# ChampiB/CBO_with_OOP

Measured on AMD Instinct MI355X. Metric: candidate-intervention acquisitions/sec (16k grid, d=3), higher is better.
Workload: dtype f64

## Files before the change

cbo_with_oop_amd/_lib.py:

```python
from __future__ import annotations

import atexit
import ctypes
import os
import threading
import weakref

import numpy as np

_HERE = os.path.dirname(os.path.abspath(__file__))
LIB_PATH = os.environ.get("CBO_HIP_LIB", os.path.join(_HERE, "libcbo_hip.so"))

c_double_p = ctypes.POINTER(ctypes.c_double)
c_int64_p = ctypes.POINTER(ctypes.c_int64)
c_int_p = ctypes.POINTER(ctypes.c_int)
c_void_pp = ctypes.POINTER(ctypes.c_void_p)

ABI_VERSION = 5
ABI_DIAG_BASE = 1000
MAX_DIM = 8
CBO_OK = 0
CBO_ERR_INVALID = -1
CBO_ERR_HIP = -2
CBO_ERR_NOT_PD = -3
# ... 79 lines not shown
                                        c_double_p, ctypes.c_int64, c_void_pp]),
    "cbo_cands_destroy": (None, [ctypes.c_void_p]),
    "cbo_cands_keep_solution": (ctypes.c_int, [ctypes.c_void_p, ctypes.c_int]),
    "cbo_gp_append": (ctypes.c_int, [ctypes.c_void_p, c_double_p, ctypes.c_double, ctypes.c_double, ctypes.c_double,
                                     c_int_p]),
    "cbo_acq_sweep": (ctypes.c_int, [ctypes.c_void_p, ctypes.c_void_p, ctypes.c_double, ctypes.c_int,
                                     ctypes.c_double, ctypes.c_double, c_double_p, c_double_p, c_double_p,
                                     c_double_p, c_int64_p]),
    "cbo_gp_fit_sweep": (ctypes.c_int, [ctypes.c_void_p, ctypes.c_void_p, ctypes.c_double, ctypes.c_int,
                                        ctypes.c_double, ctypes.c_double, c_double_p, c_double_p, c_double_p,
                                        c_double_p, c_int64_p, c_int_p, c_double_p]),
    "cbo_acq_sweep_sets": (ctypes.c_int, [ctypes.c_int, c_void_pp, c_void_pp, c_double_p, ctypes.c_int, ctypes.c_double,
                                          c_double_p, c_double_p, c_int64_p]),
    "cbo_gp_fit_level": (ctypes.c_int, [ctypes.c_void_p, ctypes.c_int, c_int_p, c_double_p]),
    "cbo_comm_gather_i64": (ctypes.c_int, [ctypes.c_void_p, ctypes.c_int64, c_int64_p]),
    "cbo_comm_share_factor": (ctypes.c_int, [ctypes.c_void_p, ctypes.c_void_p, ctypes.c_int, c_int_p, ctypes.c_int,
                                              c_int_p, ctypes.c_int]),
    "cbo_gp_take_factor_slices": (ctypes.c_int, [ctypes.c_void_p, ctypes.c_void_p, ctypes.c_int, ctypes.c_int]),
    "cbo_schedule_report": (ctypes.c_int, [ctypes.c_void_p, ctypes.c_char_p, ctypes.c_int64]),
    "cbo_trial_step": (ctypes.c_int, [ctypes.c_int, c_void_pp, c_void_pp, ctypes.c_int, ctypes.c_int64, c_double_p, c_double_p,
                                      c_double_p, c_double_p, c_double_p, ctypes.c_int, ctypes.c_double, c_double_p, c_double_p,
                                      c_int64_p, c_int_p]),
    "cbo_acq_sweep_host": (ctypes.c_int, [ctypes.c_void_p, ctypes.c_int64, c_double_p, c_double_p, c_double_p,
                                          ctypes.c_double, ctypes.c_int, ctypes.c_double, ctypes.c_double,
                                          c_double_p, c_double_p, c_int64_p]),
    "cbo_argmax_sets": (ctypes.c_int, [c_double_p, ctypes.c_int, c_int_p]),
    "cbo_argmax_pairs": (ctypes.c_int, [c_double_p, c_int64_p, ctypes.c_int, c_double_p, c_int64_p]),
    "cbo_sem_create": (ctypes.c_int, [ctypes.c_void_p, ctypes.POINTER(CboSemSpec), ctypes.c_int64, ctypes.c_int,
                                      c_double_p, c_void_pp]),
    "cbo_sem_destroy": (None, [ctypes.c_void_p]),
    "cbo_sem_target": (ctypes.c_int, [ctypes.c_void_p, ctypes.c_int, ctypes.c_int64, ctypes.c_int, c_int_p,
                                      c_double_p, c_double_p]),
    "cbo_selftest_mfma": (ctypes.c_int, [ctypes.c_void_p, c_double_p]),
    "cbo_comm_unique_id": (ctypes.c_int, [ctypes.c_void_p]),
    "cbo_comm_init_rank": (ctypes.c_int, [ctypes.c_void_p, ctypes.c_int, ctypes.c_int, ctypes.c_void_p, c_void_pp]),
    "cbo_comm_init_all": (ctypes.c_int, [ctypes.c_int, c_void_pp, c_void_pp]),
    "cbo_comm_destroy": (None, [ctypes.c_void_p]),
    "cbo_comm_size": (ctypes.c_int, [ctypes.c_void_p, c_int_p, c_int_p]),
    "cbo_comm_argmax": (ctypes.c_int, [ctypes.c_void_p, ctypes.c_double, ctypes.c_int64, c_double_p, c_int64_p]),
    "cbo_comm_argmax_all": (ctypes.c_int, [ctypes.c_int, c_void_pp, c_double_p, c_int64_p, c_double_p, c_int64_p]),
    "cbo_comm_max_f64": (ctypes.c_int, [ctypes.c_void_p, ctypes.c_double, c_double_p]),
    "cbo_comm_barrier": (ctypes.c_int, [ctypes.c_void_p]),
}

_lib = None
_lock = threading.Lock()


def load():
    global _lib
    with _lock:
        if _lib is None:
            if not os.path.exists(LIB_PATH):
                raise ImportError(
                    f"{LIB_PATH} not found: build it with `make -C cbo_with_oop_amd/csrc` (or "
                    f"`python -c 'import __graft_entry__ as g; g.build()'`).  There is no CPU fallback.")
            lib = ctypes.CDLL(LIB_PATH)
            for name, (restype, argtypes) in SIGNATURES.items():
                fn = getattr(lib, name)
                fn.restype = restype
                fn.argtypes = argtypes
            version = lib.cbo_abi_version()
            if version >= ABI_DIAG_BASE and os.environ.get("CBO_HIP_ALLOW_DIAG") != "1":
                raise ImportError(
                    f"{LIB_PATH} is a timing-only diagnostic build (cbo_abi_version() = {version}): its results may be "
                    f"wrong by construction.  Measurement scripts opt in with CBO_HIP_ALLOW_DIAG=1.")
# ... 131 lines not shown
```

cbo_with_oop_amd/csrc/cbo_api.hip:

```cpp
#include <algorithm>
#include <atomic>
#include <cmath>
#include <cstdio>
#include <cstdlib>
#include <chrono>
#include <cstring>
#include <mutex>
#include <string>
#include <map>
#include <utility>
#include <vector>

#include "cbo_internal.h"
#include "schedule_tuner.h"

using namespace cbo;

static thread_local std::string g_err;
static std::atomic<uint64_t> g_fit_stamp{0};

static int fail(int code, const std::string &msg)
{
    g_err = msg;
    return code;
// ... 350 lines not shown
    if (c->sweep_stream) hipStreamDestroy(c->sweep_stream);
    if (c->bulk_stream) hipStreamDestroy(c->bulk_stream);
    if (c->side_stream) hipStreamDestroy(c->side_stream);
    if (c->stream) hipStreamDestroy(c->stream);
    delete c;
}

extern "C" int cbo_synchronize(cbo_ctx *c)
{
    if (!c) return fail(CBO_ERR_INVALID, "ctx is NULL");
    HIP_TRY(hipSetDevice(c->device));
    HIP_TRY(hipDeviceSynchronize());
    return CBO_OK;
}

#ifdef CBO_DIAG_KNOBS
__global__ void diag_fill_kernel(double *p, int64_t n)
{
    for (int64_t i = blockIdx.x * (int64_t)blockDim.x + threadIdx.x; i < n; i += (int64_t)gridDim.x * blockDim.x)
        p[i] = 1e-3 * (double)((i * 2654435761u) & 1023u) - 0.5;
}
extern "C" int cbo_diag_update_kernel_time(cbo_ctx *c, int n, int klen, int chunk_blocks, int half_lds, int upper, int reps,
                                           double *ms_out)
{
    if (!c || !ms_out) return fail(CBO_ERR_INVALID, "NULL argument");
    HIP_TRY(hipSetDevice(c->device));
    const int64_t lda = (int64_t)n + 80;
    double *A = nullptr;
    HIP_TRY(hipMalloc(&A, sizeof(double) * (size_t)n * (size_t)lda));
    hipLaunchKernelGGL(diag_fill_kernel, dim3(4096), dim3(256), 0, c->stream, A, (int64_t)n * lda);
    hipEvent_t a, b;
    HIP_TRY(hipEventCreate(&a));
    HIP_TRY(hipEventCreate(&b));
    launch_gemm_update(c->stream, A, lda, A, lda, A, lda, 0, klen, klen, n, n, chunk_blocks, half_lds != 0, upper != 0, nullptr);
    HIP_TRY(hipEventRecord(a, c->stream));
    for (int r = 0; r < reps; ++r)
        launch_gemm_update(c->stream, A, lda, A, lda, A, lda, 0, klen, klen, n, n, chunk_blocks, half_lds != 0, upper != 0, nullptr);
    HIP_TRY(hipEventRecord(b, c->stream));
    HIP_TRY(hipStreamSynchronize(c->stream));
    float ms = 0.f;
    HIP_TRY(hipEventElapsedTime(&ms, a, b));
    *ms_out = (double)ms / reps;
    hipEventDestroy(a);
    hipEventDestroy(b);
    hipFree(A);
    return CBO_OK;
}
#endif

extern "C" int cbo_set_profiling(cbo_ctx *c, int enabled)
{
    if (!c) return fail(CBO_ERR_INVALID, "ctx is NULL");
    c->profiling = enabled != 0;
    return CBO_OK;
}

extern "C" int cbo_reset_timers(cbo_ctx *c)
{
    if (!c) return fail(CBO_ERR_INVALID, "ctx is NULL");
    resolve_events(c);
    c->timers = cbo_timers{};
    return CBO_OK;
}

extern "C" int cbo_get_timers(cbo_ctx *c, cbo_timers *out)
{
    if (!c || !out) return fail(CBO_ERR_INVALID, "NULL argument");
    resolve_events(c);
    *out = c->timers;
    return CBO_OK;
// ... 1622 lines not shown
        const int frc = cbo_gp_fit(g, nullptr, nullptr);
        if (frc != CBO_OK) return frc;
    }
    int rc = ensure_alpha(g);
    if (rc != CBO_OK) return rc;
    const int64_t n_pad = g->n_pad;
    int64_t chunk = 0, ldv = 0;
    rc = ensure_workspaces(c, n_pad, n_pad, &chunk, &ldv);
    if (rc != CBO_OK) return rc;
    if (chunk < n_pad) return fail(CBO_ERR_UNSUPPORTED, "likelihood gradients need an n_pad x n_pad workspace (raise CBO_HIP_WORKSPACE_MB)");
    const int64_t ldw = n_pad + kLdExtra;
    const size_t w_bytes = sizeof(double) * (size_t)n_pad * (size_t)ldw;
    const size_t part_elems = (size_t)lml_grad_tiles(n_pad) * (size_t)(1 + g->d);
    if (w_bytes > c->W_bytes || part_elems > c->gpart_elems) {
        HIP_TRY(hipStreamSynchronize(c->stream));
        hipFree(c->W); hipFree(c->gpart);
        c->W = nullptr; c->gpart = nullptr; c->W_bytes = 0; c->gpart_elems = 0;
        HIP_TRY(hipMalloc(&c->W, w_bytes));
        c->W_bytes = w_bytes;
        HIP_TRY(hipMalloc(&c->gpart, sizeof(double) * part_elems));
        c->gpart_elems = part_elems;
    }
    launch_set_identity(c->stream, c->V, ldv, n_pad);
    if (prefer_right_looking(c, n_pad, n_pad)) {
        rc = enqueue_right_looking(g, c->V, ldv, n_pad, c->q, c->mu, true);
        if (rc != CBO_OK) return rc;
    } else {
        launch_trsm_strips(c->stream, g->A, g->lda, g->invDt, c->V, ldv, n_pad, n_pad, g->z, c->q, c->mu);
    }
    HIP_TRY(hipMemsetAsync(c->W, 0, w_bytes, c->stream));
    for (int k0 = 0; k0 < (int)n_pad; k0 += 256) {
        const int klen = (k0 + 256 <= (int)n_pad) ? 256 : 128;
        launch_gemm_update(c->stream, c->V, ldv, c->V, ldv, c->W, ldw, k0, klen, 0, k0 + klen, k0 + klen,
                           c->pipe_chunk_blocks, true, true);
    }
    launch_lml_grad(c->stream, g->X, g->h, g->alpha, c->W, ldw, n_pad, c->gpart, c->part_val);
    launch_lml_terms(c->stream, g->A, g->lda, n_pad, g->z, c->part_val + 16);
    HIP_TRY(hipGetLastError());
    launch_dot2(c->stream, g->alpha, g->alpha, g->n, c->part_val + 20);
    launch_sum(c->stream, c->q, g->n, c->part_val + 22);
    HIP_TRY(hipGetLastError());
    double hs[24];
    HIP_TRY(hipMemcpyAsync(hs, c->part_val, sizeof(hs), hipMemcpyDeviceToHost, c->stream));
    HIP_TRY(hipStreamSynchronize(c->stream));
    lml_outputs(g, hs, hs[16], hs[17], hs[20], hs[22], lml_out, dvariance_out, dlengthscale_out, dnoise_out);
    return CBO_OK;
}

static int ensure_reversed_factor(cbo_gp *g)
{
    cbo_ctx *c = g->ctx;
    if (!g->T) {
        HIP_TRY(hipMalloc(&g->T, sizeof(double) * (size_t)g->n_pad * (size_t)g->lda));
        HIP_TRY(hipMalloc(&g->invT, sizeof(double) * (size_t)(g->n_pad / 16) * 256));
        g->t_stamp = 0;
    }
    if (g->t_stamp != g->fit_stamp) {
        launch_reversed_factor(c->stream, g->A, g->lda, g->n_pad, g->invDt, g->T, g->lda, g->invT);
        HIP_TRY(hipGetLastError());
        g->t_stamp = g->fit_stamp;
    }
    return CBO_OK;
}

extern "C" int cbo_gp_predict_gradients(cbo_gp *g, int64_t m, const double *Xs, const double *pv_s, double *dmean_out,
                                        double *dvar_out)
{
// ... 229 lines not shown
    if (target < 0 || target >= m->spec.n_nodes) return fail(CBO_ERR_INVALID, "sem: target node out of range");
    if (n_iv < 0 || n_iv > CBO_SEM_MAX_NODES) return fail(CBO_ERR_INVALID, "sem: n_iv out of range");
    if (n_iv > 0 && (!iv_nodes || !values)) return fail(CBO_ERR_INVALID, "sem: intervention nodes/values missing");
    for (int j = 0; j < n_iv; ++j)
        if (iv_nodes[j] < 0 || iv_nodes[j] >= m->spec.n_nodes)
            return fail(CBO_ERR_INVALID, "sem: intervened node out of range");
    cbo_ctx *c = m->ctx;
    HIP_TRY(hipSetDevice(c->device));
    const int nb = sem_partial_blocks(m->n_draws);
    const int iv_cols = n_iv > 0 ? n_iv : 1;
    if (n_iv_sets > m->cap_m || iv_cols > m->cap_iv) {
        HIP_TRY(hipStreamSynchronize(c->stream));
        hipFree(m->values); hipFree(m->partial); hipFree(m->mean); hipFree(m->iv_nodes);
        m->values = m->partial = m->mean = nullptr; m->iv_nodes = nullptr; m->cap_m = 0; m->cap_iv = 0;
        const int64_t cap = n_iv_sets > m->cap_m ? n_iv_sets : m->cap_m;
        HIP_TRY(hipMalloc(&m->values, sizeof(double) * cap * CBO_SEM_MAX_NODES));
        HIP_TRY(hipMalloc(&m->partial, sizeof(double) * cap * nb));
        HIP_TRY(hipMalloc(&m->mean, sizeof(double) * cap));
        HIP_TRY(hipMalloc(&m->iv_nodes, sizeof(int) * CBO_SEM_MAX_NODES));
        m->cap_m = cap; m->cap_iv = CBO_SEM_MAX_NODES;
    }
    if (n_iv > 0) {
        HIP_TRY(hipMemcpyAsync(m->values, values, sizeof(double) * n_iv_sets * n_iv, hipMemcpyHostToDevice, c->stream));
        HIP_TRY(hipMemcpyAsync(m->iv_nodes, iv_nodes, sizeof(int) * n_iv, hipMemcpyHostToDevice, c->stream));
    }
    launch_sem_target(c->stream, m->spec, m->eps_cm, m->n_draws, target, n_iv_sets, n_iv, iv_nodes, m->iv_nodes, m->values,
                      m->partial, m->mean);
    HIP_TRY(hipGetLastError());
    HIP_TRY(hipMemcpyAsync(mean_out, m->mean, sizeof(double) * n_iv_sets, hipMemcpyDeviceToHost, c->stream));
    HIP_TRY(hipStreamSynchronize(c->stream));
    return CBO_OK;
}

extern "C" int cbo_selftest_mfma(cbo_ctx *c, double *max_abs_err_out)
{
    if (!c) return fail(CBO_ERR_INVALID, "ctx is NULL");
    HIP_TRY(hipSetDevice(c->device));
    double err = -1.0;
    if (run_mfma_selftest(c->stream, &err) != 0) return fail(CBO_ERR_HIP, "mfma selftest launch failed");
    if (max_abs_err_out) *max_abs_err_out = err;
    if (err != 0.0) return fail(CBO_ERR_HIP, "fp64 MFMA lane map differs from what the kernels assume");
    double err32 = -1.0;
    if (run_mfma_f32_selftest(c->stream, &err32) != 0) return fail(CBO_ERR_HIP, "f32 mfma selftest launch failed");
    if (max_abs_err_out) *max_abs_err_out = err32 > err ? err32 : err;
    if (err32 != 0.0) return fail(CBO_ERR_HIP, "fp32 MFMA lane map differs from what the kernels assume");
    return CBO_OK;
}
```

cbo_with_oop_amd/csrc/cbo_internal.h:

```cpp
#pragma once

#include <hip/hip_runtime.h>
#include <cstddef>
#include <cstdint>
#include <string>
#include <vector>

#include "cbo_hip.h"

namespace cbo {

typedef double d4 __attribute__((ext_vector_type(4)));
typedef double d2 __attribute__((ext_vector_type(2)));

#if defined(__HIP_DEVICE_COMPILE__) || defined(__HIPCC__)
typedef __attribute__((address_space(3))) void *lds_ptr_t;
__device__ __forceinline__ void glds16(const double *gsrc, unsigned lds_dst)
{
    unsigned keep;
    asm volatile("s_mov_b32 %0, m0\n\ts_mov_b32 m0, %2\n\ts_nop 0\n\tglobal_load_lds_dwordx4 %1, off\n\ts_mov_b32 m0, %0"
                 : "=&s"(keep)
                 : "v"(gsrc), "s"(lds_dst)
                 : "memory");
}
// ... 92 lines not shown
void set_panel_form_override(int form);
void sweep_pipe_pair(const SweepPipe &pipe, hipStream_t chain, const double *A, int64_t lda, const double *invDt,
                     int64_t n_pad, int p, int r0, int klen);
void sweep_pipe_tail(const SweepPipe &pipe, hipStream_t chain, const double *A, int64_t lda, const double *invDt,
                     int64_t n_pad, int pairs_done);
void launch_backsolve(hipStream_t s, const double *A, int64_t lda, int64_t n_pad, const double *invDt, double *alpha);
void launch_forward_vec(hipStream_t s, const double *A, int64_t lda, int64_t n_pad, const double *invDt, double *w,
                        double *out);
void launch_gather_column(hipStream_t s, const double *V, int64_t ldv, int64_t n_pad, double *dst);
bool launch_backsolve_chain(hipStream_t s, const double *A, int64_t lda, int64_t n_pad, const double *invDt,
                            const double *src, int64_t src_stride, double *work, double *out, int *info);
bool launch_forward_chain(hipStream_t s, const double *A, int64_t lda, int64_t n_pad, const double *invDt, const double *w,
                          double *out, int *info);
void launch_backsolve_vec(hipStream_t s, const double *A, int64_t lda, int64_t n_pad, const double *invDt,
                          const double *src, int64_t src_stride, double *work, double *out);
void launch_pred_gradients(hipStream_t s, const PointSet &X, int64_t n_pad, const PointSet &C, int64_t c_begin,
                           int64_t cols, int64_t m, const KernelHyper &h, const double *inv_ls_dev, const double *alpha,
                           const double *W, int64_t ldw, double *dmean, double *dvar);
void launch_reversed_factor(hipStream_t s, const double *A, int64_t lda, int64_t n_pad, const double *invDt, double *T,
                            int64_t ldt, double *invT);
void launch_reverse_rows(hipStream_t s, const double *V, int64_t ldv, int64_t n_pad, int64_t cols, double *W, int64_t ldw);
void launch_dot2(hipStream_t s, const double *a, const double *b, int64_t n, double *out2);
void launch_sum(hipStream_t s, const double *a, int64_t n, double *out);
void launch_expand_interventions(hipStream_t s, const double *observed, int64_t n_obs, int d, const double *values, int n_iv,
                                 const int *iv_index, int64_t m, double *raw);

void launch_trsm_strips(hipStream_t s, const double *U, int64_t ldu, const double *invDt, double *V, int64_t ldv,
                        int64_t n, int64_t m_pad, const double *z, double *q, double *mu, bool accumulate = false,
                        bool half_lds = false);
void launch_trsm_update(hipStream_t s, const double *U, int64_t ldu, double *V, int64_t ldv, int k0, int klen,
                        int i0_begin, int i0_end, int64_t m_pad, int chunk_blocks, bool half_lds = true);
void launch_gemm_update(hipStream_t s, const double *U, int64_t ldu, const double *V, int64_t ldv, double *C,
                        int64_t ldc, int k0, int klen, int i0_begin, int i0_end, int64_t m_pad, int chunk_blocks,
                        bool half_lds, bool upper_only, const int *skip_if = nullptr);

struct cbo_small_set {
    const double *xs, *sq, *sv, *pm, *y;
    const double *cxs, *csq, *csv, *cpm, *cpv;
    int64_t ld, cld, m, index_offset;
    int n, d, zero_diag, task;
    double variance, lengthscale, noise_var, diag_add, y_best, ei_jitter, cost;
    int ard, pad_;
    const double *stage, *stage_ls;
    double *raw, *pv;
};
struct cbo_small_result {
    double best_val;
    int64_t best_idx;
    int info;
    int seq;
};
size_t small_sets_scratch_doubles(int n_sets, int blocks_per_set);
constexpr int kSmallLmlTerms = 1 + CBO_MAX_DIM + 4;
struct cbo_small_lml_result {
    double terms[kSmallLmlTerms];
    int info, seq;
};
size_t small_lml_scratch_doubles();
void launch_small_lml(hipStream_t s, const cbo_small_set &st, double *scratch, int *info, cbo_small_lml_result *out, int seq);
size_t mid_lml_scratch_doubles();
void launch_small_lml_batch(hipStream_t s, const cbo_small_set *sets, int n_models, double *scratch, int64_t stride,
                            int *info, cbo_small_lml_result *out, int seq);
void launch_small_sets(hipStream_t s, const cbo_small_set *sets, int n_sets, int blocks_per_set, double *scratch,
                       double *part_val, int64_t *part_idx, int *info, int *ticket, cbo_small_result *out, int seq);

struct AcqParams {
    double variance, noise_var, y_best, ei_jitter, cost;
// ... 35 lines not shown
```

cbo_with_oop_amd/csrc/kernels_chol.hip:

```cpp
#include <hip/hip_ext.h>
#include <climits>
#include <atomic>
#include <cstdlib>
#include <cstring>
#include <vector>

#include "cbo_device.h"

namespace cbo {

#define MFMA_F64(a, b, c) __builtin_amdgcn_mfma_f64_16x16x4f64((a), (b), (c), 0, 0, 0)

__device__ __forceinline__ double readlane_f64(double v, int lane)
{
    const int lo = __builtin_amdgcn_readlane(__double2loint(v), lane);
    const int hi = __builtin_amdgcn_readlane(__double2hiint(v), lane);
    return __hiloint2double(hi, lo);
}

constexpr int kDiagLd = 144;

struct Diag2Shared {
    double S[128][kDiagLd];
    double Yt[2][16][16];
// ... 1742 lines not shown
        if (fused && n2 > 0) launch_panel_fused(s, A, lda, r0, rcol, invDt, info_dev, zvec, n2, flags + 2 * (r0 / 128), spin_limit, nullptr, split_now);
        else launch_diag(r0);
        if (n2 <= 0) { sweep_rows(r0, 128); break; }
        if (fused) {}
        else if (lean_panel) launch_panel_trsm(s, A, lda, r0, r0 + 128, n2, invDt, info_dev);
        else
        launch_trsm_strips(s, A + (int64_t)r0 * lda + r0, lda, invDt + (int64_t)(r0 / 16) * 256,
                           A + (int64_t)r0 * lda + r0 + 128, lda, 128, n2, nullptr, nullptr, nullptr, false, half_lds);
        launch_syrk_rows(s, A, lda, r0, 128, n2, rcol, info_dev);
        const int r1 = r0 + 128;
        const int n3 = (int)n_pad - r1 - 128;
        const bool bulk = n3 > 256;
        const bool gemm_form = bulk && n3 - 256 >= syrk_gemm_rows;
        const bool carried = bulk && (fused || lean_panel);
        const hipEvent_t ev_panel = (carried && gemm_form && (!grouped || last_of_group)) ? events[2 * k] : nullptr;
        const hipEvent_t ev_rows = (carried && !gemm_form) ? events[2 * k] : nullptr;
        if (fused && n3 > 0)
            launch_panel_fused(s, A, lda, r1, rcol, invDt, info_dev, zvec, n3, flags + 2 * (r1 / 128), spin_limit, ev_panel, split_now);
        else launch_diag(r1);
        if (n3 <= 0) { sweep_rows(r0, 256); break; }
        if (fused) {}
        else if (lean_panel) launch_panel_trsm(s, A, lda, r1, r1 + 128, n3, invDt, info_dev, ev_panel);
        else
        launch_trsm_strips(s, A + (int64_t)r1 * lda + r1, lda, invDt + (int64_t)(r1 / 16) * 256,
                           A + (int64_t)r1 * lda + r1 + 128, lda, 128, n3, nullptr, nullptr, nullptr, false, half_lds);
        sweep_rows(r0, 256);
        if (grouped) {
            const int S = 256 * group_pairs, g0 = group_g0, n = (int)n_pad;
            const int next_end = (g0 + 2 * S < n) ? g0 + 2 * S : n;
            if (last_of_group) {
                hipStreamWaitEvent(side, events[2 * k], 0);
                const int a_end = (g0 + 3 * S < n) ? g0 + 3 * S : n;
                launch_gemm_update(side, A, lda, A, lda, A, lda, g0, S, next_end, a_end, n_pad + kRhsCols, syrk_gemm_chunk,
                                   syrk_gemm_half, true, info_dev);
                hipEventRecord(events[2 * group_first_k + 1], side);
                pending_big_a = 2 * group_first_k + 1;
                if (a_end < n)
                    launch_gemm_update(side, A, lda, A, lda, A, lda, g0, S, a_end, n, n_pad + kRhsCols, syrk_gemm_chunk,
                                       syrk_gemm_half, true, info_dev);
                hipEventRecord(events[2 * k + 1], side);
                pending = 2 * k + 1;
            }
            launch_syrk_rows(s, A, lda, r0, 256, n3, rcol, info_dev, 256, nullptr);
            if (first_of_group && pending_big_a >= 0) hipStreamWaitEvent(s, events[pending_big_a], 0);
            launch_gemm_update(s, A, lda, A, lda, A, lda, r0, 256, r0 + 512, next_end, n_pad + kRhsCols, syrk_gemm_chunk,
                               syrk_gemm_half, true, info_dev);
            --group_left;
            continue;
        }
        const int prev = pending;
        auto launch_bulk = [&] {
            if (!carried) hipEventRecord(events[2 * k], s);
            hipStreamWaitEvent(side, events[2 * k], 0);
            if (gemm_form)
                launch_gemm_update(side, A, lda, A, lda, A, lda, r0, 256, r0 + 256 + 256, (int)n_pad, n_pad + kRhsCols,
                                   syrk_gemm_chunk, syrk_gemm_half, true, info_dev);
            else
                launch_syrk(side, A, lda, r0, 256, n3, rcol, 4, n3 / 64, info_dev);
            hipEventRecord(events[2 * k + 1], side);
            pending = 2 * k + 1;
        };
        if (gemm_form) launch_bulk();
        if (prev >= 0) hipStreamWaitEvent(s, events[prev], 0);
        launch_syrk_rows(s, A, lda, r0, 256, n3, rcol, info_dev, 256, ev_rows);
        if (bulk && !gemm_form) launch_bulk();
    }
    hipEventRecord(events[2 * np + 1], side);
    hipStreamWaitEvent(s, events[2 * np + 1], 0);
    if (pipe && pipe->tail_begin < (int)n_pad) sweep_pipe_tail(*pipe, s, A, lda, invDt, n_pad, pair);
}

__global__ __launch_bounds__(256) void backsolve_step_kernel(const double *__restrict__ A, int64_t lda,
                                                             const double *__restrict__ invDt, int blk, double *zt,
                                                             double *__restrict__ alpha)
{
    __shared__ double zs[128];
    __shared__ double al[128];
    const int tid = threadIdx.x;
    const int lane = tid & 63, wave = tid >> 6;
    const int b0 = blk * 128;
    if (tid < 128) zs[tid] = zt[b0 + tid];
    __syncthreads();
    for (int s = 7; s >= 0; --s) {
        const int o = 16 * s;
        if (tid < 64) {
            const int i = tid >> 2, part = tid & 3;
            const double *Y = invDt + (int64_t)(b0 / 16 + s) * 256;
            double acc = 0.0;
#pragma unroll
// ... 320 lines not shown
```

cbo_with_oop_amd/csrc/kernels_trsm.hip:

```cpp
#include <cstdlib>
#include <type_traits>

#include "cbo_internal.h"

namespace cbo {

#define MFMA_F64(a, b, c) __builtin_amdgcn_mfma_f64_16x16x4f64((a), (b), (c), 0, 0, 0)

#define SCHED_DS(n) __builtin_amdgcn_sched_group_barrier(0x100, (n), 0)
#define SCHED_MFMA(n) __builtin_amdgcn_sched_group_barrier(0x008, (n), 0)
#define SCHED_VMEM(n) __builtin_amdgcn_sched_group_barrier(0x010, (n), 0)

constexpr int kRB = 128;
constexpr int kT = kRB / 16;
constexpr int kLdsLd = kRB + 16;
constexpr int kNBuf = 3;
template <int KB>
struct StageGeom {
    static constexpr int kA = KB * kLdsLd;
    static constexpr int kB = 4 * KB * 16;
    static constexpr int kRA = KB / 4;
    static constexpr int kParts = KB / 8;
    static constexpr int kDma = 3 * kParts;
    static constexpr int kKS = KB / 4;
// ... 1151 lines not shown
                        macc += __shfl_xor(macc, 32);
                        qtot += qacc;
                        mtot += macc;
                        qacc = 0.0;
                        macc = 0.0;
                    }
                    PSTAMP(2); PSTAMP_NEXT(); buf = (buf == 2) ? 0 : buf + 1;
                }
            }
        };
        diag_phase(0, std::true_type{});
        for (int i0 = kPB; i0 < n; i0 += kPB) {
            const int nst = i0 / kPKB;
            regular_stage(i0, std::true_type{});
            for (int j = 1; j < nst; ++j) regular_stage(i0, std::false_type{});
            diag_phase(i0, std::false_type{});
        }
        asm volatile("s_waitcnt vmcnt(0)" ::: "memory");
        __builtin_amdgcn_s_barrier();

        if (SWEEP && H == 1 && kq == 0) {
            q_out[colw + lc] = qtot;
            mu_out[colw + lc] = mtot;
        }
    };
    if (h == 0) run(std::integral_constant<int, 0>{});
    else run(std::integral_constant<int, 1>{});
#undef PSTAMP
#undef PSTAMP_NEXT
}

constexpr int kAccMoves = kT * 4;

template <int KB>
__global__ __launch_bounds__(256) void trsm_update_kernel(const double *__restrict__ U, int64_t ldu,
                                                          const double *V, int64_t ldv, double *C, int64_t ldc, int k0,
                                                          int klen, int i0_begin, int i0_end, int chunk_rows,
                                                          int upper_only, const int *__restrict__ skip_if)
{
    if (skip_if && __builtin_nontemporal_load(skip_if) != 0) return;
    using G = StageGeom<KB>;
    constexpr int kA = G::kA, kB = G::kB, kRA = G::kRA, kParts = G::kParts, kDma = G::kDma, kKS = G::kKS;
    __shared__ __align__(16) double lds[kNBuf * (kA + kB)];

    const int tid = threadIdx.x;
#ifdef CBO_DIAG_KNOBS
    const unsigned long long upd_t0 = __builtin_amdgcn_s_memtime();
    const unsigned long long upd_r0 = __builtin_amdgcn_s_memrealtime();
    const int upd_id = (int)(blockIdx.y * gridDim.x + blockIdx.x);
    const bool upd_probe = tid == 0 && blockIdx.x == 7 && blockIdx.y == gridDim.y / 2;
    int upd_k = 0;
#define UPD_STAMP() do { if (upd_probe && upd_k < 128) g_upd_stage[upd_k++] = __builtin_amdgcn_s_memtime(); } while (0)
#else
#define UPD_STAMP() do { } while (0)
#endif
    const int lane = tid & 63;
    const int wave = __builtin_amdgcn_readfirstlane(tid >> 6);
    const int lc = lane & 15, kq = lane >> 4;
    const int64_t colw = (int64_t)blockIdx.x * kStrip + wave * 16;
    const int ib = i0_begin + (int)blockIdx.y * chunk_rows;
    const int ie = (ib + chunk_rows < i0_end) ? ib + chunk_rows : i0_end;
    if (ib >= ie) return;
    if (upper_only && (int)blockIdx.x * kStrip + kStrip <= ib) return;
    const int nst = klen / KB;
    double *Cc = C + colw + lc;
    double *ldsB = lds + kNBuf * kA;
    const unsigned lds_byte0 = lds_byte_address(lds);
    const double *ug = U + (int64_t)(k0 + wave * kRA) * ldu + lane * 2;
    const double *vg = V + (int64_t)(k0 + (lane >> 3)) * ldv + colw + 2 * (lane & 7);
    const int64_t b_stride = 8 * ldv;

    int ci0 = ib, cj = 0;
    const double *a_src, *b_src;
    auto locate = [&]() __attribute__((always_inline)) {
        const bool past = ci0 >= ie;
        const int ai0 = past ? ie - kRB : ci0;
        const int aj = past ? nst - 1 : cj;
        a_src = ug + (int64_t)(KB * aj) * ldu + ai0;
        b_src = vg + (int64_t)(KB * aj) * ldv;
    };
    auto advance = [&]() __attribute__((always_inline)) {
        const int wrap = (cj + 1 == nst) ? 1 : 0;
        ci0 += kRB * wrap;
        cj = (cj + 1) * (1 - wrap);
        locate();
    };
    auto issue_one = [&](int buf, int part, int q) __attribute__((always_inline)) {
        if (q < 2) {
            const unsigned la = __builtin_amdgcn_readfirstlane(lds_byte0 + 8u * (unsigned)(buf * kA + (wave * kRA) * kLdsLd));
            const int p = 2 * part + q;
            glds16(a_src + (int64_t)p * ldu, la + 8u * (unsigned)(p * kLdsLd));
        } else {
            const unsigned lb = __builtin_amdgcn_readfirstlane(
                lds_byte0 + 8u * (unsigned)(kNBuf * kA + buf * kB + wave * (KB * 16)));
            glds16(b_src + part * b_stride, lb + 8u * (unsigned)(part * 128));
        }
    };
    auto issue_part = [&](int buf, int part) __attribute__((always_inline)) {
#pragma unroll
        for (int q = 0; q < 3; ++q) issue_one(buf, part, q);
    };

    d4 acc[kT], accn[kT];
#pragma unroll
    for (int t = 0; t < kT; ++t)
#pragma unroll
        for (int r = 0; r < 4; ++r) acc[t][r] = -Cc[(int64_t)(ib + 16 * t + kq + 4 * r) * ldc];

    UPD_STAMP();
    locate();
#pragma unroll
    for (int part = 0; part < kParts; ++part) issue_part(0, part);
    advance();
#pragma unroll
    for (int part = 0; part < kParts; ++part) issue_part(1, part);
    advance();
    UPD_STAMP();

    int buf = 0;
    int boundary = 0;
    for (int i0 = ib; i0 < ie; i0 += kRB) {
        double af[2][kT], bf[2];
        bool deferred = false;
        for (int j = 0; j < nst; ++j) {
            asm volatile("s_waitcnt lgkmcnt(0)" ::: "memory");
            if (boundary) asm volatile("s_waitcnt vmcnt(%0)" ::"n"(kDma + kAccMoves) : "memory");
            else asm volatile("s_waitcnt vmcnt(%0)" ::"n"(kDma) : "memory");
            __builtin_amdgcn_s_barrier();
            UPD_STAMP();
            boundary = (boundary > 0) ? boundary - 1 : 0;
            if (j == 0 && i0 + kRB < ie) {
#pragma unroll
                for (int t = 0; t < kT; ++t)
#pragma unroll
                    for (int r = 0; r < 4; ++r) accn[t][r] = -Cc[(int64_t)(i0 + kRB + 16 * t + kq + 4 * r) * ldc];
                asm volatile("" ::: "memory");
            }
            __builtin_amdgcn_sched_barrier(0);
            const int bnext = (buf >= 1) ? buf - 1 : 2;
            const double *abase = lds + buf * kA + kq * kLdsLd + lc;
            const double *bbase = ldsB + buf * kB + wave * (KB * 16) + kq * 16 + lc;
#pragma unroll
            for (int t = 0; t < kT; ++t) {
                if (deferred) acc[t] = MFMA_F64(af[1][t], bf[1], acc[t]);
                if (t < kT / 2) {
                    af[0][2 * t] = abase[32 * t];
                    af[0][2 * t + 1] = abase[32 * t + 16];
                } else if (t == kT / 2) {
                    bf[0] = bbase[0];
                }
                __builtin_amdgcn_sched_barrier(0);
            }
#pragma unroll
            for (int jj = 0; jj < kKS - 1; ++jj) {
                const double *an = abase + 4 * (jj + 1) * kLdsLd;
#pragma unroll
                for (int t = 0; t < kT; ++t) {
                    acc[t] = MFMA_F64(af[jj & 1][t], bf[jj & 1], acc[t]);
                    if (t < kT / 2) {
                        af[(jj + 1) & 1][2 * t] = an[32 * t];
                        af[(jj + 1) & 1][2 * t + 1] = an[32 * t + 16];
                    } else if (t == kT / 2) {
                        bf[(jj + 1) & 1] = bbase[4 * (jj + 1) * 16];
                    } else if (jj < kParts) {
                        issue_one(bnext, jj, t - (kT / 2 + 1));
                    } else if (jj == kParts && t == kT / 2 + 1) {
                        advance();
                    }
                    __builtin_amdgcn_sched_barrier(0);
                }
            }
            deferred = true;
            buf = (buf == 2) ? 0 : buf + 1;
        }
#pragma unroll
        for (int t = 0; t < kT; ++t) acc[t] = MFMA_F64(af[1][t], bf[1], acc[t]);
        UPD_STAMP();
#pragma unroll
        for (int t = 0; t < kT; ++t)
#pragma unroll
            for (int r = 0; r < 4; ++r) Cc[(int64_t)(i0 + 16 * t + kq + 4 * r) * ldc] = -acc[t][r];
        asm volatile("" ::: "memory");
        UPD_STAMP();
#pragma unroll
        for (int t = 0; t < kT; ++t) acc[t] = accn[t];
        boundary = 2;
    }
    asm volatile("s_waitcnt vmcnt(0)" ::: "memory");
    __builtin_amdgcn_s_barrier();
#ifdef CBO_DIAG_KNOBS
    UPD_STAMP();
    if (tid == 0 && upd_id < 65536) {
        unsigned hw, xcc;
        asm volatile("s_getreg_b32 %0, hwreg(HW_REG_HW_ID)" : "=s"(hw));
        asm volatile("s_getreg_b32 %0, hwreg(HW_REG_XCC_ID)" : "=s"(xcc));
        g_upd_wg[5 * upd_id] = upd_t0;
        g_upd_wg[5 * upd_id + 1] = __builtin_amdgcn_s_memtime();
        g_upd_wg[5 * upd_id + 2] = (unsigned long long)hw | ((unsigned long long)xcc << 32);
        g_upd_wg[5 * upd_id + 3] = upd_r0;
        g_upd_wg[5 * upd_id + 4] = __builtin_amdgcn_s_memrealtime();
    }
#endif
#undef UPD_STAMP
}

void launch_trsm_strips(hipStream_t s, const double *U, int64_t ldu, const double *invDt, double *V, int64_t ldv,
                        int64_t n, int64_t m_pad, const double *z, double *q, double *mu, bool accumulate,
                        bool half_lds)
{
    if (n <= 0 || m_pad <= 0) return;
    const dim3 grid((unsigned)(m_pad / kStrip));
    const int acc = accumulate ? 1 : 0;
    if (half_lds) {
        if (q != nullptr)
            hipLaunchKernelGGL((trsm_strip_kernel<true, 16>), grid, dim3(256), 0, s, U, ldu, invDt, V, ldv, (int)n, z, q, mu, acc);
        else
            hipLaunchKernelGGL((trsm_strip_kernel<false, 16>), grid, dim3(256), 0, s, U, ldu, invDt, V, ldv, (int)n, z, q, mu, 0);
        return;
    }
    static const bool pairs = [] {
        const char *e = getenv("CBO_HIP_STRIP_FORM");
        return !(e && atoi(e) == 8);
    }();
    if (pairs && n >= kPB && n % kPB == 0) {
#ifdef CBO_DIAG_KNOBS
        static const int pair_mask = [] {
            const char *e = getenv("CBO_HIP_STRIP_MASK");
            return e ? atoi(e) : 0;
        }();
        const int acc = (accumulate ? 1 : 0) | (pair_mask << 8);
#endif
        if (q != nullptr)
            hipLaunchKernelGGL((trsm_pair_kernel<true>), grid, dim3(512), 0, s, U, ldu, invDt, V, ldv, (int)n, z, q, mu, acc);
        else
            hipLaunchKernelGGL((trsm_pair_kernel<false>), grid, dim3(512), 0, s, U, ldu, invDt, V, ldv, (int)n, z, q, mu, 0);
        return;
    }
    if (q != nullptr)
        hipLaunchKernelGGL((trsm_strip8_kernel<true>), grid, dim3(512), 0, s, U, ldu, invDt, V, ldv, (int)n, z, q, mu, acc);
    else
        hipLaunchKernelGGL((trsm_strip8_kernel<false>), grid, dim3(512), 0, s, U, ldu, invDt, V, ldv, (int)n, z, q, mu, 0);
}

void launch_trsm_update(hipStream_t s, const double *U, int64_t ldu, double *V, int64_t ldv, int k0, int klen,
                        int i0_begin, int i0_end, int64_t m_pad, int chunk_blocks, bool half_lds)
{
    launch_gemm_update(s, U, ldu, V, ldv, V, ldv, k0, klen, i0_begin, i0_end, m_pad, chunk_blocks, half_lds, false, nullptr);
}

void launch_gemm_update(hipStream_t s, const double *U, int64_t ldu, const double *V, int64_t ldv, double *C,
                        int64_t ldc, int k0, int klen, int i0_begin, int i0_end, int64_t m_pad, int chunk_blocks,
                        bool half_lds, bool upper_only, const int *skip_if)
{
    if (i0_begin >= i0_end || m_pad <= 0 || klen <= 0) return;
    const int chunk_rows = chunk_blocks * kRB;
    const unsigned chunks = (unsigned)((i0_end - i0_begin + chunk_rows - 1) / chunk_rows);
    const dim3 grid((unsigned)(m_pad / kStrip), chunks);
    const int up = upper_only ? 1 : 0;
    if (!half_lds)
        hipLaunchKernelGGL(trsm_update_kernel<32>, grid, dim3(256), 0, s, U, ldu, V, ldv, C, ldc, k0, klen, i0_begin,
                           i0_end, chunk_rows, up, skip_if);
    else
        hipLaunchKernelGGL(trsm_update_kernel<16>, grid, dim3(256), 0, s, U, ldu, V, ldv, C, ldc, k0, klen, i0_begin,
                           i0_end, chunk_rows, up, skip_if);
}

__global__ void mfma_selftest_kernel(const double *A, const double *B, double *C)
{
    const int l = threadIdx.x;
    d4 acc = {0.0, 0.0, 0.0, 0.0};
    for (int k0 = 0; k0 < 16; k0 += 4)
        acc = MFMA_F64(A[(l & 15) * 16 + k0 + (l >> 4)], B[(k0 + (l >> 4)) * 16 + (l & 15)], acc);
    d4 acc2 = {0.0, 0.0, 0.0, 0.0};
    for (int kk = 0; kk < 4; ++kk) acc2 = MFMA_F64(A[(l & 15) * 16 + 4 * kk + (l >> 4)], acc[kk], acc2);
    for (int r = 0; r < 4; ++r) {
        C[((l >> 4) + 4 * r) * 16 + (l & 15)] = acc[r];
        C[256 + ((l >> 4) + 4 * r) * 16 + (l & 15)] = acc2[r];
    }
}

int run_mfma_selftest(hipStream_t s, double *max_err)
{
    double hA[256], hB[256], hC[512], ref[256], ref2[256];
    for (int i = 0; i < 16; ++i)
        for (int j = 0; j < 16; ++j) {
            hA[i * 16 + j] = (double)((i * 7 + j * 3) % 11 - 5);
            hB[i * 16 + j] = (double)((i * 5 + j * 13 + 1) % 17 - 8);
        }
    for (int i = 0; i < 16; ++i)
        for (int j = 0; j < 16; ++j) {
            double acc = 0.0;
            for (int k = 0; k < 16; ++k) acc += hA[i * 16 + k] * hB[k * 16 + j];
            ref[i * 16 + j] = acc;
        }
    for (int i = 0; i < 16; ++i)
        for (int j = 0; j < 16; ++j) {
// ... 27 lines not shown
```

include/cbo_hip.h:

```cpp
#ifndef CBO_HIP_H
#define CBO_HIP_H

#include <stdint.h>

#ifdef __cplusplus
extern "C" {
#endif

#define CBO_HIP_ABI_VERSION 5
#define CBO_HIP_ABI_DIAG_BASE 1000
#define CBO_MAX_DIM 8

typedef enum cbo_status {
    CBO_OK = 0,
    CBO_ERR_INVALID = -1,
    CBO_ERR_HIP = -2,
    CBO_ERR_NOT_PD = -3,
    CBO_ERR_NONPOS_DIAG = -4,
    CBO_ERR_NOT_FITTED = -5,
    CBO_ERR_UNSUPPORTED = -6,
    CBO_ERR_NO_DEVICE = -7,
    CBO_ERR_COMM = -8
} cbo_status;

// ... 117 lines not shown
int cbo_comm_size(const cbo_comm *comm, int *world_out, int *rank_out);
int cbo_comm_argmax(cbo_comm *comm, double val, int64_t idx, double *best_val, int64_t *best_idx);
int cbo_comm_argmax_all(int n, cbo_comm *const *comms, const double *vals, const int64_t *idxs, double *best_val,
                        int64_t *best_idx);
int cbo_comm_max_f64(cbo_comm *comm, double value, double *max_out);
int cbo_comm_barrier(cbo_comm *comm);
int cbo_comm_gather_i64(cbo_comm *comm, int64_t value, int64_t *out);
int cbo_comm_share_factor(cbo_comm *comm, cbo_gp *gp, int level, const int *owners, int n_owners,
                          const int *needers, int n_needers);
int cbo_gp_take_factor_slices(cbo_gp *dst, cbo_gp *src, int level, int n_owners);

#define CBO_SEM_MAX_NODES 16
#define CBO_SEM_MAX_TERMS 64
enum cbo_sem_fn { CBO_FN_ID = 0, CBO_FN_SQUARE = 1, CBO_FN_EXP = 2, CBO_FN_COS = 3, CBO_FN_SIN = 4 };
typedef struct cbo_sem_spec {
    int n_nodes;
    int eps_index[CBO_SEM_MAX_NODES];
    int term_begin[CBO_SEM_MAX_NODES + 1];
    int term_parent[CBO_SEM_MAX_TERMS];
    int term_fn[CBO_SEM_MAX_TERMS];
    double term_a[CBO_SEM_MAX_TERMS];
    double term_c[CBO_SEM_MAX_TERMS];
} cbo_sem_spec;
typedef struct cbo_sem cbo_sem;

int cbo_sem_create(cbo_ctx *ctx, const cbo_sem_spec *spec, int64_t n_samples, int n_eps,
                   const double *eps , cbo_sem **out);
void cbo_sem_destroy(cbo_sem *sem);
int cbo_sem_target(cbo_sem *sem, int target, int64_t m, int n_iv, const int *iv_nodes,
                   const double *values , double *mean_out );

int cbo_selftest_mfma(cbo_ctx *ctx, double *max_abs_err_out);

#ifdef __cplusplus
}
#endif
#endif
```

Before: 3.059 million.

## Add 64x32 per-wave tile form to the GEMM/TRSM update kernel

Templates the update kernel on a wave-column count so each wave can own a 64x32 block of the C tile instead of 128x16. This cuts LDS fragment reads per MFMA step (fewer A reads, two B reads) and reshuffles where the DMA issue slots fall in the schedule. The TRSM update path defaults to the new form, while bulk Cholesky/LML updates keep the old form unless an environment variable is set. A self-test entry point is added to check the new shape.

```diff
diff --git a/cbo_with_oop_amd/_lib.py b/cbo_with_oop_amd/_lib.py
--- a/cbo_with_oop_amd/_lib.py
+++ b/cbo_with_oop_amd/_lib.py
@@ -135,6 +135,9 @@
     "cbo_sem_target": (ctypes.c_int, [ctypes.c_void_p, ctypes.c_int, ctypes.c_int64, ctypes.c_int, c_int_p,
                                       c_double_p, c_double_p]),
     "cbo_selftest_mfma": (ctypes.c_int, [ctypes.c_void_p, c_double_p]),
+    "cbo_selftest_gemm_update": (ctypes.c_int, [ctypes.c_void_p, ctypes.c_int, ctypes.c_int, ctypes.c_int64, ctypes.c_int64,
+                                                 c_double_p, c_double_p, c_double_p] + [ctypes.c_int] * 5
+                                                + [ctypes.c_int64] + [ctypes.c_int] * 3),
     "cbo_comm_unique_id": (ctypes.c_int, [ctypes.c_void_p]),
     "cbo_comm_init_rank": (ctypes.c_int, [ctypes.c_void_p, ctypes.c_int, ctypes.c_int, ctypes.c_void_p, c_void_pp]),
     "cbo_comm_init_all": (ctypes.c_int, [ctypes.c_int, c_void_pp, c_void_pp]),
diff --git a/cbo_with_oop_amd/csrc/cbo_api.hip b/cbo_with_oop_amd/csrc/cbo_api.hip
--- a/cbo_with_oop_amd/csrc/cbo_api.hip
+++ b/cbo_with_oop_amd/csrc/cbo_api.hip
@@ -406,10 +406,12 @@
     hipEvent_t a, b;
     HIP_TRY(hipEventCreate(&a));
     HIP_TRY(hipEventCreate(&b));
-    launch_gemm_update(c->stream, A, lda, A, lda, A, lda, 0, klen, klen, n, n, chunk_blocks, half_lds != 0, upper != 0, nullptr);
+    launch_gemm_update(c->stream, A, lda, A, lda, A, lda, 0, klen, klen, n, n, chunk_blocks, half_lds != 0, upper != 0, nullptr,
+                           update_wave_cols());
     HIP_TRY(hipEventRecord(a, c->stream));
     for (int r = 0; r < reps; ++r)
-        launch_gemm_update(c->stream, A, lda, A, lda, A, lda, 0, klen, klen, n, n, chunk_blocks, half_lds != 0, upper != 0, nullptr);
+        launch_gemm_update(c->stream, A, lda, A, lda, A, lda, 0, klen, klen, n, n, chunk_blocks, half_lds != 0, upper != 0, nullptr,
+                           update_wave_cols());
     HIP_TRY(hipEventRecord(b, c->stream));
     HIP_TRY(hipStreamSynchronize(c->stream));
     float ms = 0.f;
@@ -2098,7 +2100,7 @@
     for (int k0 = 0; k0 < (int)n_pad; k0 += 256) {
         const int klen = (k0 + 256 <= (int)n_pad) ? 256 : 128;
         launch_gemm_update(c->stream, c->V, ldv, c->V, ldv, c->W, ldw, k0, klen, 0, k0 + klen, k0 + klen,
-                           c->pipe_chunk_blocks, true, true);
+                           c->pipe_chunk_blocks, true, true, nullptr, bulk_update_wave_cols());
     }
     launch_lml_grad(c->stream, g->X, g->h, g->alpha, c->W, ldw, n_pad, c->gpart, c->part_val);
     launch_lml_terms(c->stream, g->A, g->lda, n_pad, g->z, c->part_val + 16);
@@ -2394,6 +2396,42 @@
     return CBO_OK;
 }
 
+extern "C" int cbo_selftest_gemm_update(cbo_ctx *c, int wave_cols, int half_lds, int64_t rows, int64_t ld, const double *U,
+                                        const double *V, double *C, int c_is_v, int k0, int klen, int i0_begin, int i0_end,
+                                        int64_t m_pad, int chunk_blocks, int upper_only, int skip)
+{
+    if (!c || !U || !V || !C) return fail(CBO_ERR_INVALID, "NULL argument");
+    const int kb = half_lds ? 16 : 32;
+    if ((wave_cols != 1 && wave_cols != 2) || rows <= 0 || ld <= 0 || k0 < 0 || klen < 2 * kb || klen % kb != 0 ||
+        k0 + klen > rows || i0_begin < 0 || i0_end > rows || i0_end > ld || i0_begin >= i0_end ||
+        (i0_end - i0_begin) % 128 != 0 || m_pad <= 0 || m_pad % kStrip != 0 || m_pad > ld || chunk_blocks < 1 ||
+        (c_is_v && i0_begin < k0 + klen))
+        return fail(CBO_ERR_INVALID, "gemm update self test: shape out of the kernel's domain");
+    HIP_TRY(hipSetDevice(c->device));
+    const size_t bytes = sizeof(double) * (size_t)rows * (size_t)ld;
+    double *dU = nullptr, *dV = nullptr, *dC = nullptr;
+    int *dskip = nullptr;
+    const int skip_val = skip ? 1 : 0;
+    int rc = CBO_OK;
+    if (hipMalloc(&dU, bytes) != hipSuccess || hipMalloc(&dV, bytes) != hipSuccess ||
+        (!c_is_v && hipMalloc(&dC, bytes) != hipSuccess) || hipMalloc(&dskip, sizeof(int)) != hipSuccess) {
+        rc = fail(CBO_ERR_HIP, "gemm update self test: device allocation failed");
+    } else {
+        double *out = c_is_v ? dV : dC;
+        hipMemcpyAsync(dU, U, bytes, hipMemcpyHostToDevice, c->stream);
+        hipMemcpyAsync(dV, c_is_v ? C : V, bytes, hipMemcpyHostToDevice, c->stream);
+        if (!c_is_v) hipMemcpyAsync(dC, C, bytes, hipMemcpyHostToDevice, c->stream);
+        hipMemcpyAsync(dskip, &skip_val, sizeof(int), hipMemcpyHostToDevice, c->stream);
+        launch_gemm_update(c->stream, dU, ld, dV, ld, out, ld, k0, klen, i0_begin, i0_end, m_pad, chunk_blocks,
+                           half_lds != 0, upper_only != 0, dskip, wave_cols);
+        hipMemcpyAsync(C, out, bytes, hipMemcpyDeviceToHost, c->stream);
+        if (hipStreamSynchronize(c->stream) != hipSuccess || hipGetLastError() != hipSuccess)
+            rc = fail(CBO_ERR_HIP, "gemm update self test failed");
+    }
+    hipFree(dU); hipFree(dV); hipFree(dC); hipFree(dskip);
+    return rc;
+}
+
 extern "C" int cbo_selftest_mfma(cbo_ctx *c, double *max_abs_err_out)
 {
     if (!c) return fail(CBO_ERR_INVALID, "ctx is NULL");
diff --git a/cbo_with_oop_amd/csrc/cbo_internal.h b/cbo_with_oop_amd/csrc/cbo_internal.h
--- a/cbo_with_oop_amd/csrc/cbo_internal.h
+++ b/cbo_with_oop_amd/csrc/cbo_internal.h
@@ -148,7 +148,9 @@
                         int i0_begin, int i0_end, int64_t m_pad, int chunk_blocks, bool half_lds = true);
 void launch_gemm_update(hipStream_t s, const double *U, int64_t ldu, const double *V, int64_t ldv, double *C,
                         int64_t ldc, int k0, int klen, int i0_begin, int i0_end, int64_t m_pad, int chunk_blocks,
-                        bool half_lds, bool upper_only, const int *skip_if = nullptr);
+                        bool half_lds, bool upper_only, const int *skip_if = nullptr, int wave_cols = 1);
+int update_wave_cols();
+int bulk_update_wave_cols();
 
 struct cbo_small_set {
     const double *xs, *sq, *sv, *pm, *y;
diff --git a/cbo_with_oop_amd/csrc/kernels_chol.hip b/cbo_with_oop_amd/csrc/kernels_chol.hip
--- a/cbo_with_oop_amd/csrc/kernels_chol.hip
+++ b/cbo_with_oop_amd/csrc/kernels_chol.hip
@@ -1798,19 +1798,19 @@
                 hipStreamWaitEvent(side, events[2 * k], 0);
                 const int a_end = (g0 + 3 * S < n) ? g0 + 3 * S : n;
                 launch_gemm_update(side, A, lda, A, lda, A, lda, g0, S, next_end, a_end, n_pad + kRhsCols, syrk_gemm_chunk,
-                                   syrk_gemm_half, true, info_dev);
+                                   syrk_gemm_half, true, info_dev, bulk_update_wave_cols());
                 hipEventRecord(events[2 * group_first_k + 1], side);
                 pending_big_a = 2 * group_first_k + 1;
                 if (a_end < n)
                     launch_gemm_update(side, A, lda, A, lda, A, lda, g0, S, a_end, n, n_pad + kRhsCols, syrk_gemm_chunk,
-                                       syrk_gemm_half, true, info_dev);
+                                       syrk_gemm_half, true, info_dev, bulk_update_wave_cols());
                 hipEventRecord(events[2 * k + 1], side);
                 pending = 2 * k + 1;
             }
             launch_syrk_rows(s, A, lda, r0, 256, n3, rcol, info_dev, 256, nullptr);
             if (first_of_group && pending_big_a >= 0) hipStreamWaitEvent(s, events[pending_big_a], 0);
             launch_gemm_update(s, A, lda, A, lda, A, lda, r0, 256, r0 + 512, next_end, n_pad + kRhsCols, syrk_gemm_chunk,
-                               syrk_gemm_half, true, info_dev);
+                               syrk_gemm_half, true, info_dev, bulk_update_wave_cols());
             --group_left;
             continue;
         }
@@ -1820,7 +1820,7 @@
             hipStreamWaitEvent(side, events[2 * k], 0);
             if (gemm_form)
                 launch_gemm_update(side, A, lda, A, lda, A, lda, r0, 256, r0 + 256 + 256, (int)n_pad, n_pad + kRhsCols,
-                                   syrk_gemm_chunk, syrk_gemm_half, true, info_dev);
+                                   syrk_gemm_chunk, syrk_gemm_half, true, info_dev, bulk_update_wave_cols());
             else
                 launch_syrk(side, A, lda, r0, 256, n3, rcol, 4, n3 / 64, info_dev);
             hipEventRecord(events[2 * k + 1], side);
diff --git a/cbo_with_oop_amd/csrc/kernels_trsm.hip b/cbo_with_oop_amd/csrc/kernels_trsm.hip
--- a/cbo_with_oop_amd/csrc/kernels_trsm.hip
+++ b/cbo_with_oop_amd/csrc/kernels_trsm.hip
@@ -1207,7 +1207,7 @@
 
 constexpr int kAccMoves = kT * 4;
 
-template <int KB>
+template <int KB, int WC>
 __global__ __launch_bounds__(256) void trsm_update_kernel(const double *__restrict__ U, int64_t ldu,
                                                           const double *V, int64_t ldv, double *C, int64_t ldc, int k0,
                                                           int klen, int i0_begin, int i0_end, int chunk_rows,
@@ -1233,12 +1233,18 @@
     const int wave = __builtin_amdgcn_readfirstlane(tid >> 6);
     const int lc = lane & 15, kq = lane >> 4;
     const int64_t colw = (int64_t)blockIdx.x * kStrip + wave * 16;
+    static_assert(WC == 1 || WC == 2, "a wave owns 128 x 16 or 64 x 32 of the C tile");
+    constexpr int kRT = kT / WC;
+    constexpr int kReads = kRT + WC;
+    constexpr int kReadSlots = (kReads + 1) / 2;
+    static_assert(kReadSlots + 3 <= kT, "the DMA of a part rides in the slots after the reads");
+    const int cg = wave % (4 / WC), rg = wave / (4 / WC);
     const int ib = i0_begin + (int)blockIdx.y * chunk_rows;
     const int ie = (ib + chunk_rows < i0_end) ? ib + chunk_rows : i0_end;
     if (ib >= ie) return;
     if (upper_only && (int)blockIdx.x * kStrip + kStrip <= ib) return;
     const int nst = klen / KB;
-    double *Cc = C + colw + lc;
+    double *Cc = C + (int64_t)blockIdx.x * kStrip + 16 * WC * cg + (int64_t)(16 * kRT * rg) * ldc + lc;
     double *ldsB = lds + kNBuf * kA;
     const unsigned lds_byte0 = lds_byte_address(lds);
     const double *ug = U + (int64_t)(k0 + wave * kRA) * ldu + lane * 2;
@@ -1280,7 +1286,7 @@
 #pragma unroll
     for (int t = 0; t < kT; ++t)
 #pragma unroll
-        for (int r = 0; r < 4; ++r) acc[t][r] = -Cc[(int64_t)(ib + 16 * t + kq + 4 * r) * ldc];
+        for (int r = 0; r < 4; ++r) acc[t][r] = -Cc[(int64_t)(ib + 16 * (t / WC) + kq + 4 * r) * ldc + 16 * (t % WC)];
 
     UPD_STAMP();
     locate();
@@ -1295,7 +1301,7 @@
     int buf = 0;
     int boundary = 0;
     for (int i0 = ib; i0 < ie; i0 += kRB) {
-        double af[2][kT], bf[2];
+        double af[2][kRT], bf[2][WC];
         bool deferred = false;
         for (int j = 0; j < nst; ++j) {
             asm volatile("s_waitcnt lgkmcnt(0)" ::: "memory");
@@ -1308,38 +1314,38 @@
 #pragma unroll
                 for (int t = 0; t < kT; ++t)
 #pragma unroll
-                    for (int r = 0; r < 4; ++r) accn[t][r] = -Cc[(int64_t)(i0 + kRB + 16 * t + kq + 4 * r) * ldc];
+                    for (int r = 0; r < 4; ++r)
+                        accn[t][r] = -Cc[(int64_t)(i0 + kRB + 16 * (t / WC) + kq + 4 * r) * ldc + 16 * (t % WC)];
                 asm volatile("" ::: "memory");
             }
             __builtin_amdgcn_sched_barrier(0);
             const int bnext = (buf >= 1) ? buf - 1 : 2;
-            const double *abase = lds + buf * kA + kq * kLdsLd + lc;
-            const double *bbase = ldsB + buf * kB + wave * (KB * 16) + kq * 16 + lc;
+            const double *abase = lds + buf * kA + kq * kLdsLd + lc + 16 * kRT * rg;
+            const double *bbase = ldsB + buf * kB + (WC * cg) * (KB * 16) + kq * 16 + lc;
+            auto read_frag = [&](int h, int jj, int e) __attribute__((always_inline)) {
+                if (e < kRT) af[h][e] = abase[4 * jj * kLdsLd + 16 * e];
+                else bf[h][e - kRT] = bbase[(e - kRT) * (KB * 16) + 4 * jj * 16];
+            };
 #pragma unroll
             for (int t = 0; t < kT; ++t) {
-                if (deferred) acc[t] = MFMA_F64(af[1][t], bf[1], acc[t]);
-                if (t < kT / 2) {
-                    af[0][2 * t] = abase[32 * t];
-                    af[0][2 * t + 1] = abase[32 * t + 16];
-                } else if (t == kT / 2) {
-                    bf[0] = bbase[0];
+                if (deferred) acc[t] = MFMA_F64(af[1][t / WC], bf[1][t % WC], acc[t]);
+                if (t < kReadSlots) {
+                    read_frag(0, 0, 2 * t);
+                    if (2 * t + 1 < kReads) read_frag(0, 0, 2 * t + 1);
                 }
                 __builtin_amdgcn_sched_barrier(0);
             }
 #pragma unroll
             for (int jj = 0; jj < kKS - 1; ++jj) {
-                const double *an = abase + 4 * (jj + 1) * kLdsLd;
 #pragma unroll
                 for (int t = 0; t < kT; ++t) {
-                    acc[t] = MFMA_F64(af[jj & 1][t], bf[jj & 1], acc[t]);
-                    if (t < kT / 2) {
-                        af[(jj + 1) & 1][2 * t] = an[32 * t];
-                        af[(jj + 1) & 1][2 * t + 1] = an[32 * t + 16];
-                    } else if (t == kT / 2) {
-                        bf[(jj + 1) & 1] = bbase[4 * (jj + 1) * 16];
+                    acc[t] = MFMA_F64(af[jj & 1][t / WC], bf[jj & 1][t % WC], acc[t]);
+                    if (t < kReadSlots) {
+                        read_frag((jj + 1) & 1, jj + 1, 2 * t);
+                        if (2 * t + 1 < kReads) read_frag((jj + 1) & 1, jj + 1, 2 * t + 1);
                     } else if (jj < kParts) {
-                        issue_one(bnext, jj, t - (kT / 2 + 1));
-                    } else if (jj == kParts && t == kT / 2 + 1) {
+                        if (t - kReadSlots < 3) issue_one(bnext, jj, t - kReadSlots);
+                    } else if (jj == kParts && t == kReadSlots) {
                         advance();
                     }
                     __builtin_amdgcn_sched_barrier(0);
@@ -1349,12 +1355,12 @@
             buf = (buf == 2) ? 0 : buf + 1;
         }
 #pragma unroll
-        for (int t = 0; t < kT; ++t) acc[t] = MFMA_F64(af[1][t], bf[1], acc[t]);
+        for (int t = 0; t < kT; ++t) acc[t] = MFMA_F64(af[1][t / WC], bf[1][t % WC], acc[t]);
         UPD_STAMP();
 #pragma unroll
         for (int t = 0; t < kT; ++t)
 #pragma unroll
-            for (int r = 0; r < 4; ++r) Cc[(int64_t)(i0 + 16 * t + kq + 4 * r) * ldc] = -acc[t][r];
+            for (int r = 0; r < 4; ++r) Cc[(int64_t)(i0 + 16 * (t / WC) + kq + 4 * r) * ldc + 16 * (t % WC)] = -acc[t][r];
         asm volatile("" ::: "memory");
         UPD_STAMP();
 #pragma unroll
@@ -1417,26 +1423,51 @@
         hipLaunchKernelGGL((trsm_strip8_kernel<false>), grid, dim3(512), 0, s, U, ldu, invDt, V, ldv, (int)n, z, q, mu, 0);
 }
 
+int update_wave_cols()
+{
+    static const int wc = [] {
+        const char *e = getenv("CBO_HIP_UPDATE_FORM");
+        return (e && atoi(e) == 1) ? 1 : 2;
+    }();
+    return wc;
+}
+
+int bulk_update_wave_cols()
+{
+    static const int wc = [] {
+        const char *e = getenv("CBO_HIP_BULK_UPDATE_FORM");
+        return (e && atoi(e) == 2) ? 2 : 1;
+    }();
+    return wc;
+}
+
 void launch_trsm_update(hipStream_t s, const double *U, int64_t ldu, double *V, int64_t ldv, int k0, int klen,
                         int i0_begin, int i0_end, int64_t m_pad, int chunk_blocks, bool half_lds)
 {
-    launch_gemm_update(s, U, ldu, V, ldv, V, ldv, k0, klen, i0_begin, i0_end, m_pad, chunk_blocks, half_lds, false, nullptr);
+    launch_gemm_update(s, U, ldu, V, ldv, V, ldv, k0, klen, i0_begin, i0_end, m_pad, chunk_blocks, half_lds, false, nullptr,
+                       update_wave_cols());
 }
 
 void launch_gemm_update(hipStream_t s, const double *U, int64_t ldu, const double *V, int64_t ldv, double *C,
                         int64_t ldc, int k0, int klen, int i0_begin, int i0_end, int64_t m_pad, int chunk_blocks,
-                        bool half_lds, bool upper_only, const int *skip_if)
+                        bool half_lds, bool upper_only, const int *skip_if, int wave_cols)
 {
     if (i0_begin >= i0_end || m_pad <= 0 || klen <= 0) return;
     const int chunk_rows = chunk_blocks * kRB;
     const unsigned chunks = (unsigned)((i0_end - i0_begin + chunk_rows - 1) / chunk_rows);
     const dim3 grid((unsigned)(m_pad / kStrip), chunks);
     const int up = upper_only ? 1 : 0;
-    if (!half_lds)
-        hipLaunchKernelGGL(trsm_update_kernel<32>, grid, dim3(256), 0, s, U, ldu, V, ldv, C, ldc, k0, klen, i0_begin,
+    if (!half_lds && wave_cols == 2)
+        hipLaunchKernelGGL((trsm_update_kernel<32, 2>), grid, dim3(256), 0, s, U, ldu, V, ldv, C, ldc, k0, klen, i0_begin,
+                           i0_end, chunk_rows, up, skip_if);
+    else if (!half_lds)
+        hipLaunchKernelGGL((trsm_update_kernel<32, 1>), grid, dim3(256), 0, s, U, ldu, V, ldv, C, ldc, k0, klen, i0_begin,
+                           i0_end, chunk_rows, up, skip_if);
+    else if (wave_cols == 2)
+        hipLaunchKernelGGL((trsm_update_kernel<16, 2>), grid, dim3(256), 0, s, U, ldu, V, ldv, C, ldc, k0, klen, i0_begin,
                            i0_end, chunk_rows, up, skip_if);
     else
-        hipLaunchKernelGGL(trsm_update_kernel<16>, grid, dim3(256), 0, s, U, ldu, V, ldv, C, ldc, k0, klen, i0_begin,
+        hipLaunchKernelGGL((trsm_update_kernel<16, 1>), grid, dim3(256), 0, s, U, ldu, V, ldv, C, ldc, k0, klen, i0_begin,
                            i0_end, chunk_rows, up, skip_if);
 }
 
diff --git a/include/cbo_hip.h b/include/cbo_hip.h
--- a/include/cbo_hip.h
+++ b/include/cbo_hip.h
@@ -173,6 +173,10 @@
 
 int cbo_selftest_mfma(cbo_ctx *ctx, double *max_abs_err_out);
 
+int cbo_selftest_gemm_update(cbo_ctx *ctx, int wave_cols, int half_lds, int64_t rows, int64_t ld, const double *U,
+                             const double *V, double *C, int c_is_v, int k0, int klen, int i0_begin, int i0_end,
+                             int64_t m_pad, int chunk_blocks, int upper_only, int skip);
+
 #ifdef __cplusplus
 }
 #endif
```

After: 3.066 million, median of 6. No clear change (+0.2%).
